# quantumjot/sequitr

Hardware: AMD Instinct MI355X
Metric: segmented Mpixels/sec on 512x512 tiles; IoU vs reference (higher is better)
Workload: dtype f32; 1 GPU; U-Net 2-class inference, launches of 32 512x512x1 tiles, fp32 (BASELINE.json configs[1]: filters 16-32-64-128-256, eltwise_mul bridge); logits + uint8 argmax mask; one 32-tile batch per GPU per step; tiles_this_rank=32

## Files before the change

### sequitr_amd/csrc/sq_common.h

```cpp
#pragma once
#include <hip/hip_runtime.h>
#include <stdint.h>
#include <stdio.h>
#include "../../include/sequitr_hip.h"

typedef float f32x4 __attribute__((ext_vector_type(4)));

#define SQ_NOT_MINE 1

void sq_set_error(const char *fmt, ...);

#define SQ_REQUIRE(cond, ...)            \
    do {                                 \
        if (!(cond)) {                   \
            sq_set_error(__VA_ARGS__);   \
            return SQ_EINVAL;            \
        }                                \
    } while (0)

int sq_plan_bf16_kc(int Cin);
int sq_plan_bf16_bn(int64_t ntiles, int Cout, bool pn, bool mos);
int sq_plan_mosaic_splitk(int Nimg, int h, int w, int Cin, int Cout, int R, int Cc, bool have_ws, int64_t workspace_bytes);
int sq_plan_f32_bn(int64_t ntiles, int Cout);
bool sq_plan_f32_stage32(int bn, int KS, int KC, int Cin, bool concat);
bool sq_plan_l0_takes(int mode, int cout, int act, int H, int W, bool concat, int head_c, bool pooled);
int sq_wgrad_f32_plan(int N, int H, int W, int Cin, int Cout, int K, int64_t *out);

#define SQ_ALIGNED16(p) ((((uintptr_t)(p)) & 15u) == 0)

#define SQ_REQUIRE_ALIGNED(p)                                     \
    do {                                                          \
        if (!SQ_ALIGNED16(p)) {                                   \
            sq_set_error("%s: pointer %s not 16-byte aligned", __func__, #p); \
            return SQ_EALIGN;                                     \
        }                                                         \
    } while (0)

static inline int sq_check_launch(const char *what) {
    hipError_t e = hipGetLastError();
    if (e != hipSuccess) {
        sq_set_error("%s: launch failed: %s", what, hipGetErrorString(e));
        return SQ_ELAUNCH;
    }
    return SQ_OK;
}

__device__ __forceinline__ float sq_act(float v, int act) {
    if (act == SQ_ACT_RELU) return v > 0.0f ? v : 0.0f;
    if (act == SQ_ACT_LEAKY) return v > 0.0f ? v : 0.2f * v;
    return v;
}

__device__ __forceinline__ unsigned sq_xcd_remap(unsigned bid, unsigned nblk) {
    const unsigned q = nblk >> 3, r = nblk & 7u, xcd = bid & 7u, k = bid >> 3;
    const unsigned base = xcd < r ? xcd * (q + 1) : r * (q + 1) + (xcd - r) * q;
    return base + k;
}

struct SqDropKey { unsigned s1, s2; };
__device__ __forceinline__ SqDropKey sq_dropout_key(unsigned seed, const int *__restrict__ step) {
    if (step) seed += (unsigned)step[0] * 0x9E3779B9u;
    SqDropKey k;
    k.s1 = seed * 0x9E3779B1u + 0x7F4A7C15u;
    k.s2 = (seed ^ 0x68E31DA4u) * 0x85EBCA6Bu;
    k.s2 ^= k.s2 >> 13;
    return k;
}
__device__ __forceinline__ unsigned sq_dropout_thr16(float rate) { return (unsigned)(rate * 65536.0f); }
__device__ __forceinline__ unsigned sq_dropout_keep4(SqDropKey k, unsigned q, unsigned thr16) {
    unsigned h = q + k.s1;
    h ^= h >> 16; h *= 0x7FEB352Du; h = h ^ (h >> 15) ^ k.s2; h *= 0x846CA68Bu; h ^= h >> 16;
    unsigned g = (h ^ 0x5BD1E995u) * 0x2C1B3C6Du;
    g ^= g >> 15;
    return (unsigned)((h & 0xFFFFu) >= thr16) | ((unsigned)((h >> 16) >= thr16) << 1) |
           ((unsigned)((g & 0xFFFFu) >= thr16) << 2) | ((unsigned)((g >> 16) >= thr16) << 3);
}

template <int MAXC>
__device__ __forceinline__ float sq_wce_pixel(const float (&zc)[MAXC], const float (&yc)[MAXC], int C, float wp, float g,
                                              float *__restrict__ dz) {
#pragma clang fp contract(off)
    float m = -INFINITY, yt = 0.f, dot = 0.f;
#pragma unroll
    for (int c = 0; c < MAXC; ++c)
        if (c < C) {
            m = zc[c] > m ? zc[c] : m;
            yt += yc[c];
            dot = __builtin_fmaf(yc[c], zc[c], dot);
        }
    float s = 0.f;
#pragma unroll
    for (int c = 0; c < MAXC; ++c)
        if (c < C) s += expf(zc[c] - m);
    const float lse = m + logf(s);
    if (dz) {
#pragma unroll
        for (int c = 0; c < MAXC; ++c)
            if (c < C) dz[c] = g * (expf(zc[c] - lse) * yt - yc[c]);
    }
    return wp * (lse * yt - dot);
}

__device__ __forceinline__ float sq_group_reduce(const float *__restrict__ p, size_t stride, int nblk, int g, int G) {
    float s = 0.f;
    int b = g;
    for (; b + 7 * G < nblk; b += 8 * G) {
        float v[8];
#pragma unroll
        for (int u = 0; u < 8; ++u) v[u] = p[(size_t)(b + u * G) * stride];
#pragma unroll
        for (int u = 0; u < 8; ++u) s += v[u];
    }
    for (; b < nblk; b += G) s += p[(size_t)b * stride];
    for (int m = G >> 1; m > 0; m >>= 1) s += __shfl_xor(s, m);
    return s;
}
static inline int sq_group_size(int nblk) {
    int G = 1;
    while (G < 64 && G * 2 <= nblk) G *= 2;
    return G;
}
```

### sequitr_amd/csrc/sq_conv_epi.h

```cpp
#pragma once
#include "sq_common.h"

struct SqConvEpi {
    float *pooled;
    const float *head_w;
    const float *head_b;
    float *logits;
    uint8_t *mask;
    int head_c;
    int store_y;
    const float *first_w;
    const float *first_b;
    const float *up_x;
    const float *up_w;
    const float *up_b;
    int up_bridge;
    const float *x2;
};

#define SQ_L0_NOT_MINE 1
int sq_conv_l0_launch(int mode, const float *x, const float *w, const float *bias, float *y, int N, int H, int W,
                      int cout, int act, const SqConvEpi &epi, hipStream_t st);
```

### sequitr_amd/csrc/sq_conv_f32_v2.hip

```cpp
#include <stdlib.h>
#include <type_traits>
#include "sq_common.h"
#include "sq_conv_epi.h"

#ifndef SQ_V2_FAST32
#define SQ_V2_FAST32 1
#endif
#ifndef SQ_V2_INNER
#define SQ_V2_INNER 1
#endif
#ifndef SQ_TILE_INTERLEAVE
#define SQ_TILE_INTERLEAVE 1
#endif
#ifndef SQ_STORE_PERMUTE
#define SQ_STORE_PERMUTE 0
#endif


namespace {

constexpr int TH = 16, TW = 16;

template <int BN, int KS, int KC>
struct Cfg2 {
// ... 293 lines not shown
            const float *src = xl + (((hy + 1) >> 1) * C::UP_W + ((hx + 1) >> 1)) * C::UP_PS + kk;
            f32x4 c1 = (f32x4){0.f, 0.f, 0.f, 0.f};
#pragma unroll
            for (int s8 = 0; s8 < 8; ++s8) c1 = __builtin_amdgcn_mfma_f32_16x16x4f32(aw[s8], src[4 * s8], c1, 0, 0, 0);
            const int gy = ty * TH - 1 + hy, gx = tx * TW - 1 + hx;
            const bool inside = (unsigned)gy < (unsigned)H && (unsigned)gx < (unsigned)W;
            if (j < 81) {
                float *d = xs + (hy * C::HALO_W + hx) * C::PS + 4 * kk;
                const float u[4] = {c1[0] + upb.x, c1[1] + upb.y, c1[2] + upb.z, c1[3] + upb.w};
                const float sk[4] = {sr[blk].x, sr[blk].y, sr[blk].z, sr[blk].w};
                float m[4];
#pragma unroll
                for (int e = 0; e < 4; ++e) {
                    const float v = epi.up_bridge == SQ_BRIDGE_ADD ? u[e] + sk[e]
                                  : (epi.up_bridge == SQ_BRIDGE_MUL ? u[e] * sk[e]
                                  : (epi.up_bridge == SQ_BRIDGE_SUB ? u[e] - sk[e] : u[e]));
                    m[e] = inside ? v : 0.f;
                }
                *reinterpret_cast<float2 *>(d) = make_float2(m[0], m[1]);
                *reinterpret_cast<float2 *>(d + 2) = make_float2(m[2], m[3]);
            }
        }
    };

    f32x4 acc[4][NR];
    const float *xb_lds = xs + ((4 * wv) * C::HALO_W + li) * C::PS + kk;
    const float *wa_lds = ws + kk * C::BNS + li;

    auto load_frag = [&](int st, float (&a)[NR], float (&b)[4]) {
        constexpr int SPC = KS * KS * 4;
        const int sub = KC > 16 ? st / SPC : 0, sr = KC > 16 ? st % SPC : st;
        constexpr int Q = KC > 16 ? 4 : KC / 4;
        const int tap = sr / Q, s = sr % Q;
        const int ky = tap / KS, kx = tap % KS;
        const int ch = sub * 16 + s * 4;
#pragma unroll
        for (int nb = 0; nb < NR; ++nb)
            a[nb] = wa_lds[(tap * KC + ch) * C::BNS + ((nb * 16) ^ ((kk & 1) ? C::WSWZ : 0))];
#pragma unroll
        for (int r = 0; r < 4; ++r) b[r] = xb_lds[((r + ky) * C::HALO_W + kx) * C::PS + ch];
    };

    const float slope = act == SQ_ACT_LEAKY ? 0.2f : 1.0f;
    const bool is_relu = act == SQ_ACT_RELU;
    auto actk = [&](float v, auto fastc) {
        if constexpr (decltype(fastc)::value) return __builtin_fmaxf(v, 0.0f);
        else {
            const float neg = is_relu ? 0.0f : v * slope;
            return v > 0.0f ? v : neg;
        }
    };

    float ah[4] = {0.f, 0.f, 0.f, 0.f};
    float hb[4] = {0.f, 0.f, 0.f, 0.f};
    if (epi.head_w) {
#pragma unroll
        for (int s4 = 0; s4 < 4; ++s4) ah[s4] = li < epi.head_c ? epi.head_w[(4 * s4 + kk) * epi.head_c + li] : 0.f;
        if (epi.head_b) {
#pragma unroll
            for (int q = 0; q < 4; ++q) hb[q] = q < epi.head_c ? epi.head_b[q] : 0.f;
        }
    }

#if SQ_STORE_PERMUTE
    const int st_src = (((lane & 3) << 4) | (lane >> 2)) << 2;
    const int st_px = lane >> 2, st_q = lane & 3;
#endif
    float4 bvr[NR];
#pragma unroll
    for (int nb = 0; nb < NR; ++nb) {
        const int co = n0 + nb * 16 + 4 * kk;
        bvr[nb] = (bias && co < Cout) ? *reinterpret_cast<const float4 *>(bias + co) : make_float4(0.f, 0.f, 0.f, 0.f);
    }
    const int fast_lane = (((4 * wv) * W + li) * Cout + 4 * kk) * 4;
    auto epilogue = [&](int tx, int ty, int n, auto fastc) {
        constexpr bool FAST = decltype(fastc)::value;
        auto actf = [&](float v) { return actk(v, fastc); };
        const int gx = tx * TW + li;
#pragma unroll
        for (int nb = 0; nb < NR; ++nb) {
            const int co = n0 + nb * 16 + 4 * kk;
            const float4 bv = bvr[nb];
            f32x4 o[4];
#pragma unroll
            for (int r = 0; r < 4; ++r) {
                const int gy = ty * TH + 4 * wv + r;
                o[r][0] = actf(bias ? acc[r][nb][0] + bv.x : acc[r][nb][0]);
                o[r][1] = actf(bias ? acc[r][nb][1] + bv.y : acc[r][nb][1]);
                o[r][2] = actf(bias ? acc[r][nb][2] + bv.z : acc[r][nb][2]);
                o[r][3] = actf(bias ? acc[r][nb][3] + bv.w : acc[r][nb][3]);
                if (epi.store_y) {
#if SQ_STORE_PERMUTE
                    const float t0 = __int_as_float(__builtin_amdgcn_ds_bpermute(st_src, __float_as_int(o[r][0])));
                    const float t1 = __int_as_float(__builtin_amdgcn_ds_bpermute(st_src, __float_as_int(o[r][1])));
                    const float t2 = __int_as_float(__builtin_amdgcn_ds_bpermute(st_src, __float_as_int(o[r][2])));
                    const float t3 = __int_as_float(__builtin_amdgcn_ds_bpermute(st_src, __float_as_int(o[r][3])));
                    f32x4 t = (f32x4){t0, t1, t2, t3};
                    const int sgx = tx * TW + st_px, sco = n0 + nb * 16 + 4 * st_q;
                    const bool ok = gy < H && sgx < W && sco < Cout;
                    const unsigned off = ok ? (unsigned)((((n * H + gy) * W + sgx) * Cout + sco) * 4) : OOB;
                    __builtin_amdgcn_raw_buffer_store_b128(
                        *reinterpret_cast<__attribute__((__vector_size__(4 * sizeof(unsigned)))) unsigned *>(&t),
                        yrsrc, off, 0, 0);
#else
                    unsigned off;
                    if constexpr (FAST) {
                        off = (unsigned)(fast_lane + nb * 64) + (unsigned)((((n * H + ty * TH + r) * W + tx * TW) * Cout + n0) * 4);
                    } else {
                        const bool ok = gy < H && gx < W && co < Cout;
                        off = ok ? (unsigned)((((n * H + gy) * W + gx) * Cout + co) * 4) : OOB;
                    }
                    __builtin_amdgcn_raw_buffer_store_b128(
                        *reinterpret_cast<__attribute__((__vector_size__(4 * sizeof(unsigned)))) unsigned *>(&o[r]),
                        yrsrc, off, 0, 0);
#endif
                }
                acc[r][nb] = (f32x4){0.f, 0.f, 0.f, 0.f};
            }
            if (epi.pooled) {
#pragma unroll
                for (int pr = 0; pr < 2; ++pr) {
                    float mp[4];
#pragma unroll
                    for (int j = 0; j < 4; ++j) {
                        const float a = o[2 * pr][j], b = o[2 * pr + 1][j];
                        const float v = b > a ? b : a;
                        const float u = __shfl_xor(v, 1);
                        mp[j] = u > v ? u : v;
                    }
                    const int py = (ty * TH + 4 * wv) / 2 + pr, px = gx >> 1;
                    if ((li & 1) == 0 && py < (H >> 1) && px < (W >> 1) && co < Cout)
                        *reinterpret_cast<float4 *>(epi.pooled + ((size_t)(n * (H >> 1) + py) * (W >> 1) + px) * Cout + co) =
                            make_float4(mp[0], mp[1], mp[2], mp[3]);
                }
            }
            if (epi.head_w) {
                float *hs = head_scratch + wv * (16 * C::HEAD_PS);
#pragma unroll
                for (int r = 0; r < 4; ++r) {
                    float *d = hs + li * C::HEAD_PS + 4 * kk;
                    *reinterpret_cast<float2 *>(d) = make_float2(o[r][0], o[r][1]);
                    *reinterpret_cast<float2 *>(d + 2) = make_float2(o[r][2], o[r][3]);
                    __builtin_amdgcn_wave_barrier();
                    f32x4 z = (f32x4){0.f, 0.f, 0.f, 0.f};
#pragma unroll
                    for (int s4 = 0; s4 < 4; ++s4)
                        z = __builtin_amdgcn_mfma_f32_16x16x4f32(ah[s4], hs[li * C::HEAD_PS + 4 * s4 + kk], z, 0, 0, 0);
                    __builtin_amdgcn_wave_barrier();
                    const int gy = ty * TH + 4 * wv + r;
                    if (kk == 0 && gy < H && gx < W) {
                        const size_t p = (size_t)(n * H + gy) * W + gx;
                        float best = 0.f;
                        int bi = 0;
#pragma unroll
                        for (int q = 0; q < 4; ++q)
                            if (q < epi.head_c) {
                                const float v = epi.head_b ? z[q] + hb[q] : z[q];
                                epi.logits[p * epi.head_c + q] = v;
                                if (q == 0 || v > best) { best = v; bi = q; }
                            }
                        if (epi.mask) epi.mask[p] = (uint8_t)bi;
                    }
                }
            }
        }
    };

    const int per_image = tiles_x * tiles_y;
    const int s_n = tstride / per_image, s_y = (tstride % per_image) / tiles_x, s_x = (tstride % per_image) % tiles_x;
    int ctx = t_begin % tiles_x, cty = (t_begin / tiles_x) % tiles_y, cn = t_begin / per_image;
    int ntx = ctx + s_x, nty = cty, nn = cn;
    if (ntx >= tiles_x) { ntx -= tiles_x; nty += 1; }
    nty += s_y;
    if (nty >= tiles_y) { nty -= tiles_y; nn += 1; }
    nn += s_n;
    issue(ctx, cty, cn, 0, true, true);
    __builtin_amdgcn_s_waitcnt(0x0F70);
    commit(true);
#pragma unroll
    for (int r = 0; r < 4; ++r)
#pragma unroll
        for (int nb = 0; nb < NR; ++nb) acc[r][nb] = (f32x4){0.f, 0.f, 0.f, 0.f};
    __syncthreads();
    if constexpr (FIRST) {
        first_conv(ctx, cty);
        __syncthreads();
    }
    if constexpr (UP) {
        up_conv(ctx, cty);
        __syncthreads();
    }

    int tile = t_begin, chunk = 0;
    for (int it = 0; it < nitems; ++it) {
        int ntile = tile, nchk = chunk + 1;
        if (nchk == nchunk) { nchk = 0; ntile = tile + tstride; }
        const bool has_next = it + 1 < nitems;
        const bool same = ntile == tile;
        const int itx = same ? ctx : ntx, ity = same ? cty : nty, itn = same ? cn : nn;
        if (has_next) issue(itx, ity, itn, nchk * KC, restage_w, true);

        {
            float a0[NR], b0[4], a1[NR], b1[4];
            load_frag(0, a0, b0);
            __builtin_amdgcn_s_setprio(0);
#pragma unroll
            for (int st = 0; st < C::NSTEP; st += 2) {
                if (st + 1 < C::NSTEP) load_frag(st + 1, a1, b1);
                __builtin_amdgcn_sched_barrier(0);
#pragma unroll
                for (int r = 0; r < 4; ++r)
#pragma unroll
                    for (int nb = 0; nb < NR; ++nb)
                        acc[r][nb] = __builtin_amdgcn_mfma_f32_16x16x4f32(a0[nb], b0[r], acc[r][nb], 0, 0, 0);
                __builtin_amdgcn_sched_barrier(0);
                if (st + 1 < C::NSTEP) {
                    if (st + 2 < C::NSTEP) load_frag(st + 2, a0, b0);
                    __builtin_amdgcn_sched_barrier(0);
#pragma unroll
                    for (int r = 0; r < 4; ++r)
#pragma unroll
                        for (int nb = 0; nb < NR; ++nb)
                            acc[r][nb] = __builtin_amdgcn_mfma_f32_16x16x4f32(a1[nb], b1[r], acc[r][nb], 0, 0, 0);
                    __builtin_amdgcn_sched_barrier(0);
                }
            }
            __builtin_amdgcn_s_setprio(3);
        }
        __builtin_amdgcn_s_waitcnt(0x0F70);
        if (has_next) {
            __syncthreads();
            commit(restage_w);
            if constexpr (FIRST) {
                __syncthreads();
                first_conv(itx, ity);
            }
            if constexpr (UP) {
                __syncthreads();
                up_conv(itx, ity);
            }
        }
        if (chunk == nchunk - 1) {
            const bool fast = is_relu && cty * TH + TH <= H && ctx * TW + TW <= W && n0 + BN <= Cout;
            if constexpr ((BN == 64 || (SQ_V2_FAST32 && BN == 32 && KC == 32)) && MODE == 0) {
                if (fast) epilogue(ctx, cty, cn, std::integral_constant<bool, true>{});
                else epilogue(ctx, cty, cn, std::integral_constant<bool, false>{});
            } else {
                (void)fast;
                epilogue(ctx, cty, cn, std::integral_constant<bool, false>{});
            }
        }
        if (has_next) __syncthreads();
        if (ntile != tile) {
            ctx = ntx; cty = nty; cn = nn;
            ntx += s_x;
            if (ntx >= tiles_x) { ntx -= tiles_x; nty += 1; }
            nty += s_y;
            if (nty >= tiles_y) { nty -= tiles_y; nn += 1; }
            nn += s_n;
        }
        tile = ntile;
        chunk = nchk;
    }
}

template <int BN, int KS, int KC, int MODE>
int launch_v2(const float *x, const float *w, const float *bias, float *y, int N, int H, int W, int Cin,
              int Cout, float wscale, int act, const SqConvEpi &epi, hipStream_t st) {
    using C = Cfg2<BN, KS, KC>;
    static bool attr_set = false;
    auto kern = conv_mfma_f32_v2_kernel<BN, KS, KC, MODE>;
    constexpr int lds_base = MODE == 1 ? C::LDS_BYTES_FIRST : (MODE == 2 ? C::LDS_BYTES_UP : C::LDS_BYTES);
    constexpr int lds_max = lds_base + C::HEAD_FLOATS * 4;
    const int lds = lds_base + (epi.head_w ? C::HEAD_FLOATS * 4 : 0);
    if (!attr_set) {
        if (hipFuncSetAttribute(reinterpret_cast<const void *>(kern),
                                hipFuncAttributeMaxDynamicSharedMemorySize, lds_max) != hipSuccess) {
            sq_set_error("conv_mfma_f32_v2: cannot reserve %d bytes of LDS", lds_max);
            return SQ_ELAUNCH;
        }
        attr_set = true;
    }
    const int tiles_x = (W + TW - 1) / TW, tiles_y = (H + TH - 1) / TH;
    const int ntiles = tiles_x * tiles_y * N;
    const int gy = (Cout + BN - 1) / BN;
    int want = (256 * (MODE == 2 ? 3 : C::OCC) + gy - 1) / gy;
    if (want < 1) want = 1;
    int tpb = (ntiles + want - 1) / want;
    if (tpb < 1) tpb = 1;
    const int gx = (ntiles + tpb - 1) / tpb;
    hipLaunchKernelGGL(kern, dim3(gx, gy), dim3(256), lds, st, x, w, bias, y, N, H, W, Cin, Cout,
                       wscale, act, tiles_x, tiles_y, ntiles, tpb, epi);
    return sq_check_launch("sq_conv2d_nhwc_fwd_f32(v2)");
}

template <int KS, int KC>
int dispatch_bn(const float *x, const float *w, const float *bias, float *y, int N, int H, int W, int Cin,
                int Cout, float wscale, int act, const SqConvEpi &epi, hipStream_t st) {
    const int ntiles = ((W + TW - 1) / TW) * ((H + TH - 1) / TH) * N;
    const int bn = sq_plan_f32_bn(ntiles, Cout);
    if constexpr (KS == 3 && KC == 16) {
        if (sq_plan_f32_stage32(bn, KS, KC, Cin, epi.x2 != nullptr))
            return launch_v2<32, 3, 32, false>(x, w, bias, y, N, H, W, Cin, Cout, wscale, act, epi, st);
    }
    if (bn == 64) return launch_v2<64, KS, KC, false>(x, w, bias, y, N, H, W, Cin, Cout, wscale, act, epi, st);
    if (bn == 32) return launch_v2<32, KS, KC, false>(x, w, bias, y, N, H, W, Cin, Cout, wscale, act, epi, st);
    return launch_v2<16, KS, KC, false>(x, w, bias, y, N, H, W, Cin, Cout, wscale, act, epi, st);
}

bool fits32(int N, int H, int W, int C) { return (size_t)N * H * W * (size_t)C * 4 < ((size_t)1 << 31); }

}

int sq_conv_mfma_v2(const float *x, const float *w, const float *bias, float *y, int N, int H, int W,
                    int Cin, int Cout, int K, float wscale, int act, hipStream_t st) {
    SqConvEpi epi = {};
    epi.store_y = 1;
    if (Cin == 16 && (Cout == 16 || Cout == 32) && K == 3 && wscale == 1.0f) {
        const int r = sq_conv_l0_launch(0, x, w, bias, y, N, H, W, Cout, act, epi, st);
        if (r != SQ_L0_NOT_MINE) return r;
    }
    if (Cin % 16 == 0)
        return K == 3 ? dispatch_bn<3, 16>(x, w, bias, y, N, H, W, Cin, Cout, wscale, act, epi, st)
                      : dispatch_bn<1, 16>(x, w, bias, y, N, H, W, Cin, Cout, wscale, act, epi, st);
    return K == 3 ? dispatch_bn<3, 8>(x, w, bias, y, N, H, W, Cin, Cout, wscale, act, epi, st)
                  : dispatch_bn<1, 8>(x, w, bias, y, N, H, W, Cin, Cout, wscale, act, epi, st);
}

extern "C" int sq_conv2d_concat_nhwc_fwd_f32(const float *xa, const float *xb, const float *w, const float *bias, float *y,
                                             int N, int H, int W, int Ca, int Cout, int K, int act, void *stream) {
    SQ_REQUIRE(xa && xb && w && y, "sq_conv2d_concat_nhwc_fwd_f32: null tensor pointer");
    SQ_REQUIRE(N > 0 && H > 0 && W > 0 && (K == 1 || K == 3), "sq_conv2d_concat_nhwc_fwd_f32: bad shape / K");
    SQ_REQUIRE(Ca % 16 == 0 && Ca > 0 && Cout % 4 == 0 && Cout > 0,
               "sq_conv2d_concat_nhwc_fwd_f32: channels per source %d (multiple of 16), Cout=%d (multiple of 4)", Ca, Cout);
    SQ_REQUIRE(fits32(N, H, W, 2 * Ca > Cout ? 2 * Ca : Cout), "sq_conv2d_concat_nhwc_fwd_f32: tensors must be < 2 GiB");
    SQ_REQUIRE(act >= SQ_ACT_NONE && act <= SQ_ACT_LEAKY, "sq_conv2d_concat_nhwc_fwd_f32: bad activation %d", act);
    SQ_REQUIRE_ALIGNED(xa); SQ_REQUIRE_ALIGNED(xb); SQ_REQUIRE_ALIGNED(w); SQ_REQUIRE_ALIGNED(y);
    if (bias) SQ_REQUIRE_ALIGNED(bias);
    SqConvEpi epi = {};
    epi.store_y = 1;
    epi.x2 = xb;
    hipStream_t st = reinterpret_cast<hipStream_t>(stream);
    return K == 3 ? dispatch_bn<3, 16>(xa, w, bias, y, N, H, W, 2 * Ca, Cout, 1.0f, act, epi, st)
                  : dispatch_bn<1, 16>(xa, w, bias, y, N, H, W, 2 * Ca, Cout, 1.0f, act, epi, st);
}

extern "C" int sq_conv3x3_pool_fwd_f32(const float *x, const float *w, const float *bias, float *y, float *pooled,
                                       int N, int H, int W, int Cin, int Cout, int act, void *stream) {
    SQ_REQUIRE(x && w && y && pooled, "sq_conv3x3_pool_fwd_f32: null tensor pointer");
    SQ_REQUIRE(N > 0 && H > 0 && W > 0 && H % 2 == 0 && W % 2 == 0, "sq_conv3x3_pool_fwd_f32: H, W must be even");
    SQ_REQUIRE(Cin % 16 == 0 && Cin > 0 && Cout % 4 == 0 && Cout > 0,
               "sq_conv3x3_pool_fwd_f32: Cin=%d (multiple of 16), Cout=%d (multiple of 4)", Cin, Cout);
    SQ_REQUIRE(fits32(N, H, W, Cin > Cout ? Cin : Cout), "sq_conv3x3_pool_fwd_f32: tensors must be < 2 GiB");
    SQ_REQUIRE(act >= SQ_ACT_NONE && act <= SQ_ACT_LEAKY, "sq_conv3x3_pool_fwd_f32: bad activation %d", act);
    SQ_REQUIRE_ALIGNED(x); SQ_REQUIRE_ALIGNED(w); SQ_REQUIRE_ALIGNED(y); SQ_REQUIRE_ALIGNED(pooled);
    if (bias) SQ_REQUIRE_ALIGNED(bias);
    SqConvEpi epi = {};
    epi.store_y = 1;
    epi.pooled = pooled;
    if (Cin == 16 && Cout == 16) {
        const int r = sq_conv_l0_launch(0, x, w, bias, y, N, H, W, 16, act, epi, reinterpret_cast<hipStream_t>(stream));
        if (r != SQ_L0_NOT_MINE) return r;
    }
    return dispatch_bn<3, 16>(x, w, bias, y, N, H, W, Cin, Cout, 1.0f, act, epi, reinterpret_cast<hipStream_t>(stream));
}

extern "C" int sq_conv3x3_head_fwd_f32(const float *x, const float *w, const float *bias, const float *head_w,
                                       const float *head_b, float *logits, uint8_t *mask, int N, int H, int W,
                                       int Cin, int head_c, int act, void *stream) {
    SQ_REQUIRE(x && w && head_w && logits, "sq_conv3x3_head_fwd_f32: null tensor pointer");
    SQ_REQUIRE(N > 0 && H > 0 && W > 0 && Cin % 16 == 0 && Cin > 0, "sq_conv3x3_head_fwd_f32: Cin=%d (multiple of 16)", Cin);
    SQ_REQUIRE(head_c >= 1 && head_c <= 4, "sq_conv3x3_head_fwd_f32: head_c=%d (1..4)", head_c);
    SQ_REQUIRE(fits32(N, H, W, Cin > 16 ? Cin : 16), "sq_conv3x3_head_fwd_f32: tensors must be < 2 GiB");
    SQ_REQUIRE(act >= SQ_ACT_NONE && act <= SQ_ACT_LEAKY, "sq_conv3x3_head_fwd_f32: bad activation %d", act);
    SQ_REQUIRE_ALIGNED(x); SQ_REQUIRE_ALIGNED(w);
    if (bias) SQ_REQUIRE_ALIGNED(bias);
    SqConvEpi epi = {};
    epi.store_y = 0;
    epi.head_w = head_w; epi.head_b = head_b; epi.logits = logits; epi.mask = mask; epi.head_c = head_c;
    if (Cin == 16) {
        const int r = sq_conv_l0_launch(0, x, w, bias, nullptr, N, H, W, 16, act, epi, reinterpret_cast<hipStream_t>(stream));
        if (r != SQ_L0_NOT_MINE) return r;
    }
    return launch_v2<16, 3, 16, false>(x, w, bias, nullptr, N, H, W, Cin, 16, 1.0f, act, epi,
                                       reinterpret_cast<hipStream_t>(stream));
}

extern "C" int sq_conv3x3_first_block_fwd_f32(const float *x, const float *w1, const float *b1, const float *w2,
                                              const float *b2, float *y, float *pooled, int N, int H, int W,
                                              void *stream) {
    SQ_REQUIRE(x && w1 && b1 && w2 && y, "sq_conv3x3_first_block_fwd_f32: null tensor pointer");
    SQ_REQUIRE(N > 0 && H > 0 && W > 0, "sq_conv3x3_first_block_fwd_f32: bad shape");
    SQ_REQUIRE(!pooled || (H % 2 == 0 && W % 2 == 0), "sq_conv3x3_first_block_fwd_f32: pooling needs even H, W");
    SQ_REQUIRE(fits32(N, H, W, 16), "sq_conv3x3_first_block_fwd_f32: tensors must be < 2 GiB");
    SQ_REQUIRE_ALIGNED(w2); SQ_REQUIRE_ALIGNED(y);
    if (b2) SQ_REQUIRE_ALIGNED(b2);
    if (pooled) SQ_REQUIRE_ALIGNED(pooled);
    SqConvEpi epi = {};
    epi.store_y = 1;
    epi.pooled = pooled;
    epi.first_w = w1; epi.first_b = b1;
    {
        const int r = sq_conv_l0_launch(1, x, w2, b2, y, N, H, W, 16, SQ_ACT_RELU, epi, reinterpret_cast<hipStream_t>(stream));
        if (r != SQ_L0_NOT_MINE) return r;
    }
    return launch_v2<16, 3, 16, true>(x, w2, b2, y, N, H, W, 1, 16, 1.0f, SQ_ACT_RELU, epi,
                                      reinterpret_cast<hipStream_t>(stream));
}

extern "C" int sq_convT_conv3x3_fwd_f32(const float *x_low, const float *wt, const float *bt, const float *skip,
                                        int bridge, const float *w, const float *bias, float *y, int N, int H, int W,
                                        int act, void *stream) {
    SQ_REQUIRE(x_low && wt && skip && w && y, "sq_convT_conv3x3_fwd_f32: null tensor pointer");
    SQ_REQUIRE(N > 0 && H > 0 && W > 0 && H % 2 == 0 && W % 2 == 0, "sq_convT_conv3x3_fwd_f32: H, W must be even");
    SQ_REQUIRE(bridge >= SQ_BRIDGE_NONE && bridge <= SQ_BRIDGE_SUB, "sq_convT_conv3x3_fwd_f32: bad bridge %d", bridge);
    SQ_REQUIRE(fits32(N, H, W, 16), "sq_convT_conv3x3_fwd_f32: tensors must be < 2 GiB");
    SQ_REQUIRE(act >= SQ_ACT_NONE && act <= SQ_ACT_LEAKY, "sq_convT_conv3x3_fwd_f32: bad activation %d", act);
    SQ_REQUIRE_ALIGNED(x_low); SQ_REQUIRE_ALIGNED(skip); SQ_REQUIRE_ALIGNED(w); SQ_REQUIRE_ALIGNED(y);
    if (bias) SQ_REQUIRE_ALIGNED(bias);
    if (bt) SQ_REQUIRE_ALIGNED(bt);
    SqConvEpi epi = {};
    epi.store_y = 1;
    epi.up_x = x_low; epi.up_w = wt; epi.up_b = bt; epi.up_bridge = bridge;
    {
        const int r = sq_conv_l0_launch(2, skip, w, bias, y, N, H, W, 16, act, epi, reinterpret_cast<hipStream_t>(stream));
        if (r != SQ_L0_NOT_MINE) return r;
    }
    return launch_v2<16, 3, 16, 2>(skip, w, bias, y, N, H, W, 16, 16, 1.0f, act, epi,
                                   reinterpret_cast<hipStream_t>(stream));
}
```

### sequitr_amd/csrc/sq_conv_plan.hip

```cpp
#include "sq_conv_epi.h"
#include <stdlib.h>

namespace {
constexpr int TILE = 16;
int64_t ntiles_of(int N, int H, int W) { return (int64_t)((W + TILE - 1) / TILE) * ((H + TILE - 1) / TILE) * N; }
}

int sq_plan_bf16_kc(int Cin) { return Cin % 32 == 0 ? 32 : (Cin % 16 == 0 ? 16 : 8); }

int sq_plan_bf16_bn(int64_t ntiles, int Cout, bool pn, bool mos) {
    if (pn) return Cout <= 16 ? 16 : (Cout <= 32 ? 32 : 64);
    int bn = Cout >= 64 ? 64 : (Cout > 16 ? 32 : 16);
    static const int narrow = [] { const char *e = getenv("SQ_CONV_BF16_NARROW"); return e ? atoi(e) : 1; }();
    while (narrow && bn > 16 && ntiles * ((Cout + bn - 1) / bn) < 2 * 256) bn >>= 1;
    static const int force_bn = [] { const char *e = getenv("SQ_MOS_BN"); return e ? atoi(e) : 0; }();
    if (mos && (force_bn == 16 || force_bn == 32 || force_bn == 64) && force_bn <= ((Cout + 15) / 16) * 16) bn = force_bn;
    return bn;
}

int sq_plan_mosaic_splitk(int Nimg, int h, int w, int Cin, int Cout, int R, int Cc, bool have_ws, int64_t workspace_bytes) {
    const int H = R * (h + 1), W = Cc * (w + 1);
    const int nchunk = Cin / sq_plan_bf16_kc(Cin);
    const int64_t blocks = ntiles_of(1, H, W) * ((Cout + 15) / 16);
    const int64_t slice = (int64_t)Nimg * h * w * Cout * 4;
    int S = 1;
    static const int sk_on = [] { const char *e = getenv("SQ_CONV_SPLITK"); return e ? atoi(e) : 1; }();
    if (sk_on && have_ws && Cout % 4 == 0 && blocks < 256 && nchunk >= 4)
        while (S < 8 && nchunk % (2 * S) == 0 && nchunk / (2 * S) >= 2 && blocks * S < 512 && slice * 2 * S <= workspace_bytes) S *= 2;
    static const int force_s = [] { const char *e = getenv("SQ_MOS_S"); return e ? atoi(e) : 0; }();
    if (force_s >= 1 && have_ws && nchunk % force_s == 0 && slice * force_s <= workspace_bytes) S = force_s;
    return S;
}

int sq_plan_f32_bn(int64_t ntiles, int Cout) {
    int bn = Cout >= 64 ? 64 : (Cout > 16 ? 32 : 16);
    while (bn > 16 && ntiles * ((Cout + bn - 1) / bn) < 2 * 256) bn >>= 1;
    return bn;
}

bool sq_plan_f32_stage32(int bn, int KS, int KC, int Cin, bool concat) {
    static const bool on = [] { const char *e = getenv("SQ_CONV_STAGE32"); return !(e && e[0] == '0'); }();
    return KS == 3 && KC == 16 && bn == 32 && Cin % 32 == 0 && !concat && on;
}

bool sq_plan_l0_takes(int mode, int cout, int act, int H, int W, bool concat, int head_c, bool pooled) {
    if (cout != 16 && !(cout == 32 && mode == 0 && !head_c && !pooled)) return false;
    const char *e = getenv("SQ_CONV_L0");
    if (e && e[0] == '0') return false;
    if (act != SQ_ACT_RELU || H % 16 != 0 || W % 16 != 0 || concat) return false;
    if (head_c && head_c != 2) return false;
    if (head_c && pooled) return false;
    return true;
}

extern "C" int sq_conv_plan(int family, int form, int N, int H, int W, int Cin, int Cout, int K, int act, int flags,
                            const int *mosaic, int64_t workspace_bytes, int *out) {
    SQ_REQUIRE(out, "sq_conv_plan: null out");
    SQ_REQUIRE(N > 0 && H > 0 && W > 0 && Cin > 0 && Cout > 0 && (K == 1 || K == 3), "sq_conv_plan: bad shape / K");
    SQ_REQUIRE(act >= SQ_ACT_NONE && act <= SQ_ACT_LEAKY, "sq_conv_plan: bad activation %d", act);
    out[0] = out[1] = out[2] = 0;
    out[3] = 1;
    out[4] = 0;
    if (family == SQ_PLAN_F32) {
        SQ_REQUIRE(!mosaic, "sq_conv_plan: the f32 family has no mosaic form");
        SQ_REQUIRE(Cout % 4 == 0 && (Cin % 16 == 0 || (Cin == 8 && form == SQ_PLAN_PLAIN)),
                   "sq_conv_plan: the f32 v2 kernels take Cin %% 16 == 0 (or 8, plain), Cout %% 4 == 0");
        SQ_REQUIRE(form == SQ_PLAN_PLAIN || form == SQ_PLAN_CONCAT || (form == SQ_PLAN_POOL && K == 3),
                   "sq_conv_plan: f32 form %d at K=%d does not exist", form, K);
        const bool wscale1 = !(flags & SQ_PLAN_WSCALE);
        const bool offer = form == SQ_PLAN_PLAIN ? (Cin == 16 && (Cout == 16 || Cout == 32) && K == 3 && wscale1)
                                                 : (form == SQ_PLAN_POOL && Cin == 16 && Cout == 16);
        if (offer && sq_plan_l0_takes(0, Cout, act, H, W, false, 0, form == SQ_PLAN_POOL)) {
            out[0] = Cout;
            out[1] = 16;
            out[2] = 1;
            out[4] = 1;
            return SQ_OK;
        }
        const int KC = Cin % 16 == 0 ? 16 : 8;
        const int bn = sq_plan_f32_bn(ntiles_of(N, H, W), Cout);
        const bool s32 = sq_plan_f32_stage32(bn, K, KC, Cin, form == SQ_PLAN_CONCAT);
        out[0] = bn;
        out[1] = s32 ? 32 : KC;
        out[2] = (Cout + bn - 1) / bn;
        return SQ_OK;
    }
    SQ_REQUIRE(family == SQ_PLAN_BF16 || family == SQ_PLAN_MIXED, "sq_conv_plan: bad family %d", family);
    SQ_REQUIRE(Cin % 8 == 0 && Cout % 4 == 0, "sq_conv_plan: Cin=%d (multiple of 8), Cout=%d (multiple of 4)", Cin, Cout);
    const bool bf = family == SQ_PLAN_BF16;
    int NN = N, HH = H, WW = W;
    if (mosaic) {
        SQ_REQUIRE(K == 3 && (form == SQ_PLAN_PLAIN || form == SQ_PLAN_ACTGATE), "sq_conv_plan: the mosaic forms are 3x3 plain / act-gated");
        SQ_REQUIRE(mosaic[0] > 0 && mosaic[1] > 0 && (int64_t)mosaic[0] * mosaic[1] >= N && H <= 8 && W <= 8,
                   "sq_conv_plan: mosaic of R x Cc >= Nimg cells of images up to 8 x 8");
        NN = 1;
        HH = mosaic[0] * (H + 1);
        WW = mosaic[1] * (W + 1);
        if (bf) out[3] = sq_plan_mosaic_splitk(N, H, W, Cin, Cout, mosaic[0], mosaic[1], workspace_bytes > 0, workspace_bytes);
    } else {
        switch (form) {
        case SQ_PLAN_PLAIN: case SQ_PLAN_ACTGATE: break;
        case SQ_PLAN_POOL: case SQ_PLAN_JUNCTION:
            SQ_REQUIRE(bf && K == 3, "sq_conv_plan: form %d is a 3x3 form on bf16 tensors", form); break;
        case SQ_PLAN_MASK: case SQ_PLAN_MASKGATE:
            SQ_REQUIRE(bf && K == 3 && Cout % 16 == 0, "sq_conv_plan: the mask forms are 3x3, Cout %% 16 == 0, bf16 tensors"); break;
        case SQ_PLAN_PIXELNORM:
            SQ_REQUIRE(bf && K == 3 && Cout % 8 == 0 && Cout <= 64, "sq_conv_plan: the pixel-norm form is 3x3, Cout %% 8 == 0, <= 64"); break;
        case SQ_PLAN_FIRSTBLOCK:
            SQ_REQUIRE(bf && K == 3 && Cin == 16 && Cout == 16, "sq_conv_plan: the first block is the 3x3 16 -> 16 conv"); break;
        default:
            SQ_REQUIRE(false, "sq_conv_plan: form %d does not exist in family %d", form, family);
        }
    }
    const int bn = sq_plan_bf16_bn(ntiles_of(NN, HH, WW), Cout, form == SQ_PLAN_PIXELNORM, mosaic != nullptr);
    out[0] = bn;
    out[1] = sq_plan_bf16_kc(Cin);
    out[2] = (Cout + bn - 1) / bn;
    return SQ_OK;
}
```

Before: 1646 Mpixels/s.

## Add specialized 64-wide f32 3x3 conv kernel with double-buffered halo staging

Result: no change. 1652 Mpixels/s, median of 6 (+0.4%).

```diff
diff --git a/sequitr_amd/csrc/sq_common.h b/sequitr_amd/csrc/sq_common.h
--- a/sequitr_amd/csrc/sq_common.h
+++ b/sequitr_amd/csrc/sq_common.h
@@ -24,6 +24,7 @@
 int sq_plan_f32_bn(int64_t ntiles, int Cout);
 bool sq_plan_f32_stage32(int bn, int KS, int KC, int Cin, bool concat);
 bool sq_plan_l0_takes(int mode, int cout, int act, int H, int W, bool concat, int head_c, bool pooled);
+bool sq_plan_w64_takes(int bn, int kc, int K, int N, int H, int W, int Cin, int Cout, int act, bool wscale1, bool concat);
 int sq_wgrad_f32_plan(int N, int H, int W, int Cin, int Cout, int K, int64_t *out);
 
 #define SQ_ALIGNED16(p) ((((uintptr_t)(p)) & 15u) == 0)
diff --git a/sequitr_amd/csrc/sq_conv_epi.h b/sequitr_amd/csrc/sq_conv_epi.h
--- a/sequitr_amd/csrc/sq_conv_epi.h
+++ b/sequitr_amd/csrc/sq_conv_epi.h
@@ -21,3 +21,5 @@
 #define SQ_L0_NOT_MINE 1
 int sq_conv_l0_launch(int mode, const float *x, const float *w, const float *bias, float *y, int N, int H, int W,
                       int cout, int act, const SqConvEpi &epi, hipStream_t st);
+int sq_conv_w64_launch(const float *x, const float *w, const float *bias, float *y, float *pooled, int N, int H, int W,
+                       int Cin, int Cout, hipStream_t st);
diff --git a/sequitr_amd/csrc/sq_conv_f32_v2.hip b/sequitr_amd/csrc/sq_conv_f32_v2.hip
--- a/sequitr_amd/csrc/sq_conv_f32_v2.hip
+++ b/sequitr_amd/csrc/sq_conv_f32_v2.hip
@@ -619,6 +619,8 @@
     if constexpr (KS == 3 && KC == 16) {
         if (sq_plan_f32_stage32(bn, KS, KC, Cin, epi.x2 != nullptr))
             return launch_v2<32, 3, 32, false>(x, w, bias, y, N, H, W, Cin, Cout, wscale, act, epi, st);
+        if (epi.store_y && !epi.head_w && sq_plan_w64_takes(bn, KC, KS, N, H, W, Cin, Cout, act, wscale == 1.0f, epi.x2 != nullptr))
+            return sq_conv_w64_launch(x, w, bias, y, epi.pooled, N, H, W, Cin, Cout, st);
     }
     if (bn == 64) return launch_v2<64, KS, KC, false>(x, w, bias, y, N, H, W, Cin, Cout, wscale, act, epi, st);
     if (bn == 32) return launch_v2<32, KS, KC, false>(x, w, bias, y, N, H, W, Cin, Cout, wscale, act, epi, st);
diff --git a/sequitr_amd/csrc/sq_conv_f32_w64.hip b/sequitr_amd/csrc/sq_conv_f32_w64.hip
--- /dev/null
+++ b/sequitr_amd/csrc/sq_conv_f32_w64.hip
@@ -0,0 +1,264 @@
+#include <stdlib.h>
+#include "sq_common.h"
+#include "sq_conv_epi.h"
+
+#ifndef SQ_W64_SETPRIO
+#define SQ_W64_SETPRIO 1
+#endif
+
+#ifndef SQ_W64_DBUF
+#define SQ_W64_DBUF 1
+#endif
+
+namespace {
+
+constexpr int TH = 16, TW = 16, HWD = 18, HP = HWD * HWD;
+constexpr int PS = 24;
+constexpr int XS_FLOATS = HP * PS;
+constexpr int XITEMS = HP * 4, XSLOTS = 6;
+constexpr int BN = 64, KC = 16;
+constexpr unsigned OOB = 0x80000000u;
+
+enum { EPI_STORE = 0, EPI_POOL = 1 };
+
+struct W64Args {
+    const float *x, *w, *bias;
+    float *y, *pooled;
+    int N, H, W, Cin, Cout;
+    int tiles_x, tiles_y, ntiles;
+};
+
+typedef unsigned u32x4 __attribute__((__vector_size__(4 * sizeof(unsigned))));
+
+__device__ __forceinline__ float relu(float v) { return __builtin_fmaxf(v, 0.0f); }
+
+template <int EPI>
+__global__ __launch_bounds__(256, 2) void conv_w64_kernel(const W64Args a) {
+    extern __shared__ __attribute__((aligned(16))) float smem[];
+    float *xs = smem;
+
+    const int tid = threadIdx.x, lane = tid & 63, wv = tid >> 6;
+    const int li = lane & 15, kk = lane >> 4;
+    const int H = a.H, W = a.W, Cin = a.Cin, Cout = a.Cout;
+    const int n0 = blockIdx.y * BN;
+    const int G = (int)gridDim.x;
+    const int vb = (int)sq_xcd_remap(blockIdx.x, gridDim.x);
+    if (vb >= a.ntiles) return;
+    const int t_count = (a.ntiles - vb + G - 1) / G;
+    const int nchunk = Cin / KC;
+    const int nitems = t_count * nchunk;
+    const bool restage_w = nchunk > 1;
+
+    const __amdgpu_buffer_rsrc_t xrsrc = __builtin_amdgcn_make_buffer_rsrc(
+        const_cast<float *>(a.x), 0, (int)((size_t)a.N * H * W * Cin * 4), 0x00020000);
+    const __amdgpu_buffer_rsrc_t wrsrc = __builtin_amdgcn_make_buffer_rsrc(
+        const_cast<float *>(a.w), 0, 9 * Cin * Cout * 4, 0x00020000);
+    const __amdgpu_buffer_rsrc_t yrsrc = __builtin_amdgcn_make_buffer_rsrc(
+        a.y, 0, (int)((size_t)a.N * H * W * Cout * 4), 0x00020000);
+
+    float4 xr[XSLOTS];
+    int xrel[XSLOTS], xpp[XSLOTS];
+#pragma unroll
+    for (int sl = 0; sl < XSLOTS; ++sl) {
+        const int idx = tid + sl * 256, pix = idx >> 2, q = idx & 3;
+        const int py = pix / HWD, px = pix % HWD;
+        xrel[sl] = idx < XITEMS ? ((py * W + px) * Cin + q * 4) * 4 : (int)OOB;
+        xpp[sl] = (py << 8) | px;
+    }
+    auto issue_halo = [&](int tx, int ty, int n, int cc) {
+        const int x0 = tx * TW - 1, y0 = ty * TH - 1;
+        const int base = (((n * H + y0) * W + x0) * Cin + cc) * 4;
+        const bool inner = tx > 0 && tx < a.tiles_x - 1 && ty > 0 && ty < a.tiles_y - 1;
+        if (inner) {
+#pragma unroll
+            for (int sl = 0; sl < XSLOTS; ++sl) {
+                const auto v = __builtin_amdgcn_raw_buffer_load_b128(xrsrc, xrel[sl], base, 0);
+                xr[sl] = *reinterpret_cast<const float4 *>(&v);
+            }
+        } else {
+#pragma unroll
+            for (int sl = 0; sl < XSLOTS; ++sl) {
+                const int py = xpp[sl] >> 8, px = xpp[sl] & 255;
+                const bool inb = (unsigned)(y0 + py) < (unsigned)H && (unsigned)(x0 + px) < (unsigned)W && xrel[sl] != (int)OOB;
+                const unsigned off = inb ? (unsigned)(base + xrel[sl]) : OOB;
+                const auto v = __builtin_amdgcn_raw_buffer_load_b128(xrsrc, off, 0, 0);
+                xr[sl] = *reinterpret_cast<const float4 *>(&v);
+            }
+        }
+    };
+    float *cw = xs + (tid >> 2) * PS + (tid & 3);
+    auto commit_halo = [&](int xoff) {
+#pragma unroll
+        for (int sl = 0; sl < XSLOTS; ++sl) {
+            if (sl < XSLOTS - 1 || tid < XITEMS - (XSLOTS - 1) * 256) {
+                float *d = cw + xoff + sl * 64 * PS;
+                d[0] = xr[sl].x; d[4] = xr[sl].y; d[8] = xr[sl].z; d[12] = xr[sl].w;
+            }
+        }
+    };
+
+    float af[9][4], wr[9][4];
+    int wvo[4];
+#pragma unroll
+    for (int s = 0; s < 4; ++s) wvo[s] = ((4 * s + kk) * Cout + n0 + 16 * wv + li) * 4;
+    auto issue_w = [&](int cc) {
+#pragma unroll
+        for (int t = 0; t < 9; ++t) {
+            const int soff = ((t * Cin + cc) * Cout) * 4;
+#pragma unroll
+            for (int s = 0; s < 4; ++s)
+                wr[t][s] = __builtin_bit_cast(float, __builtin_amdgcn_raw_buffer_load_b32(wrsrc, wvo[s], soff, 0));
+        }
+    };
+    auto take_w = [&]() {
+#pragma unroll
+        for (int t = 0; t < 9; ++t)
+#pragma unroll
+            for (int s = 0; s < 4; ++s) af[t][s] = wr[t][s];
+    };
+    const float4 bv = a.bias ? *reinterpret_cast<const float4 *>(a.bias + n0 + 16 * wv + 4 * kk) : make_float4(0.f, 0.f, 0.f, 0.f);
+
+    f32x4 acc[TH];
+    const float *xb0 = xs + li * PS + 4 * kk;
+    auto mfma_phase = [&](int xoff) {
+        const float *xb = xb0 + xoff;
+        float4 bq[2][3];
+#pragma unroll
+        for (int kx = 0; kx < 3; ++kx) bq[0][kx] = *reinterpret_cast<const float4 *>(xb + kx * PS);
+#if SQ_W64_SETPRIO
+        __builtin_amdgcn_s_setprio(0);
+#endif
+#pragma unroll
+        for (int h = 0; h < HWD; ++h) {
+            if (h + 1 < HWD) {
+#pragma unroll
+                for (int kx = 0; kx < 3; ++kx)
+                    bq[(h + 1) & 1][kx] = *reinterpret_cast<const float4 *>(xb + ((h + 1) * HWD + kx) * PS);
+            }
+            __builtin_amdgcn_sched_barrier(0);
+#pragma unroll
+            for (int kx = 0; kx < 3; ++kx) {
+                const float4 q = bq[h & 1][kx];
+                const float b[4] = {q.x, q.y, q.z, q.w};
+#pragma unroll
+                for (int s = 0; s < 4; ++s) {
+#pragma unroll
+                    for (int ky = 2; ky >= 0; --ky) {
+                        const int r = h - ky;
+                        if (r < 0 || r >= TH) continue;
+                        acc[r] = __builtin_amdgcn_mfma_f32_16x16x4f32(af[ky * 3 + kx][s], b[s], acc[r], 0, 0, 0);
+                    }
+                }
+            }
+            __builtin_amdgcn_sched_barrier(0);
+        }
+#if SQ_W64_SETPRIO
+        __builtin_amdgcn_s_setprio(3);
+#endif
+    };
+
+    const int Hl = H >> 1, Wl = W >> 1;
+    const __amdgpu_buffer_rsrc_t prsrc = __builtin_amdgcn_make_buffer_rsrc(
+        a.pooled, 0, EPI == EPI_POOL ? (int)((size_t)a.N * Hl * Wl * Cout * 4) : 0, 0x00020000);
+    const int yvoff = (li * Cout + n0 + 16 * wv + 4 * kk) * 4;
+    const int pvoff = ((li >> 1) * Cout + n0 + 16 * wv + 4 * kk) * 4;
+    auto epilogue = [&](int tx, int ty, int n) {
+        int yoff = yvoff + (((n * H + ty * TH) * W + tx * TW) * Cout) * 4;
+        int poff = pvoff + (((n * Hl + ty * (TH / 2)) * Wl + tx * (TW / 2)) * Cout) * 4;
+#pragma unroll
+        for (int p = 0; p < TH / 2; ++p) {
+            f32x4 o[2];
+#pragma unroll
+            for (int e = 0; e < 2; ++e) {
+                const int r = 2 * p + e;
+                o[e] = (f32x4){relu(acc[r][0] + bv.x), relu(acc[r][1] + bv.y), relu(acc[r][2] + bv.z), relu(acc[r][3] + bv.w)};
+                __builtin_amdgcn_raw_buffer_store_b128(*reinterpret_cast<const u32x4 *>(&o[e]), yrsrc, yoff, 0, 0);
+                yoff += W * Cout * 4;
+                acc[r] = (f32x4){0.f, 0.f, 0.f, 0.f};
+            }
+            if constexpr (EPI == EPI_POOL) {
+                f32x4 mp;
+#pragma unroll
+                for (int j = 0; j < 4; ++j) {
+                    const float v = __builtin_fmaxf(o[0][j], o[1][j]);
+                    const float u = __builtin_bit_cast(float, __builtin_amdgcn_mov_dpp(__builtin_bit_cast(int, v), 0xB1, 0xF, 0xF, true));
+                    mp[j] = __builtin_fmaxf(u, v);
+                }
+                __builtin_amdgcn_raw_buffer_store_b128(*reinterpret_cast<const u32x4 *>(&mp), prsrc,
+                                                       (li & 1) ? (int)OOB : poff, 0, 0);
+                poff += Wl * Cout * 4;
+            }
+        }
+    };
+
+    const int per_image = a.tiles_x * a.tiles_y;
+    const int s_n = G / per_image, s_y = (G % per_image) / a.tiles_x, s_x = (G % per_image) % a.tiles_x;
+    int ctx = vb % a.tiles_x, cty = (vb / a.tiles_x) % a.tiles_y, cn = vb / per_image;
+    int chunk = 0;
+    issue_halo(ctx, cty, cn, 0);
+    issue_w(0);
+    __builtin_amdgcn_s_waitcnt(0x0F70);
+    commit_halo(0);
+    take_w();
+    int xoff = 0;
+#pragma unroll
+    for (int r = 0; r < TH; ++r) acc[r] = (f32x4){0.f, 0.f, 0.f, 0.f};
+    __syncthreads();
+    for (int it = 0; it < nitems; ++it) {
+        const bool has_next = it + 1 < nitems;
+        const bool last_chunk = chunk == nchunk - 1;
+        int itx = ctx, ity = cty, itn = cn, nchk = chunk + 1;
+        if (last_chunk) {
+            nchk = 0;
+            itx += s_x;
+            if (itx >= a.tiles_x) { itx -= a.tiles_x; ity += 1; }
+            ity += s_y;
+            if (ity >= a.tiles_y) { ity -= a.tiles_y; itn += 1; }
+            itn += s_n;
+        }
+        if (has_next) {
+            issue_halo(itx, ity, itn, nchk * KC);
+            if (restage_w) issue_w(nchk * KC);
+        }
+        mfma_phase(xoff);
+        __builtin_amdgcn_s_waitcnt(0x0F70);
+#if SQ_W64_DBUF
+        xoff = XS_FLOATS - xoff;
+#endif
+        if (has_next) {
+#if !SQ_W64_DBUF
+            __syncthreads();
+#endif
+            commit_halo(xoff);
+            if (restage_w) take_w();
+        }
+        if (last_chunk) epilogue(ctx, cty, cn);
+        if (has_next) __syncthreads();
+        ctx = itx; cty = ity; cn = itn;
+        chunk = nchk;
+    }
+}
+
+template <int EPI>
+int launch_w64(W64Args a, hipStream_t st) {
+    a.tiles_x = a.W / TW;
+    a.tiles_y = a.H / TH;
+    a.ntiles = a.tiles_x * a.tiles_y * a.N;
+    const int gy = a.Cout / BN;
+    int want = (256 * 2 + gy - 1) / gy;
+    int tpb = (a.ntiles + want - 1) / want;
+    if (tpb < 1) tpb = 1;
+    const int gx = (a.ntiles + tpb - 1) / tpb;
+    hipLaunchKernelGGL(conv_w64_kernel<EPI>, dim3(gx, gy), dim3(256), XS_FLOATS * 4 * (SQ_W64_DBUF ? 2 : 1), st, a);
+    return sq_check_launch("conv_w64");
+}
+
+}
+
+int sq_conv_w64_launch(const float *x, const float *w, const float *bias, float *y, float *pooled, int N, int H, int W,
+                       int Cin, int Cout, hipStream_t st) {
+    W64Args a = {};
+    a.x = x; a.w = w; a.bias = bias; a.y = y; a.pooled = pooled;
+    a.N = N; a.H = H; a.W = W; a.Cin = Cin; a.Cout = Cout;
+    return pooled ? launch_w64<EPI_POOL>(a, st) : launch_w64<EPI_STORE>(a, st);
+}
diff --git a/sequitr_amd/csrc/sq_conv_plan.hip b/sequitr_amd/csrc/sq_conv_plan.hip
--- a/sequitr_amd/csrc/sq_conv_plan.hip
+++ b/sequitr_amd/csrc/sq_conv_plan.hip
@@ -1,5 +1,9 @@
 #include "sq_conv_epi.h"
 #include <stdlib.h>
+
+#ifndef SQ_W64_DEFAULT
+#define SQ_W64_DEFAULT 1
+#endif
 
 namespace {
 constexpr int TILE = 16;
@@ -51,6 +55,15 @@
     if (head_c && head_c != 2) return false;
     if (head_c && pooled) return false;
     return true;
+}
+
+bool sq_plan_w64_takes(int bn, int kc, int K, int N, int H, int W, int Cin, int Cout, int act, bool wscale1, bool concat) {
+    if (bn != 64 || kc != 16 || K != 3) return false;
+    const char *e = getenv("SQ_CONV_W64");
+    if (e ? e[0] == '0' : !SQ_W64_DEFAULT) return false;
+    if (Cin % 16 != 0 || Cout % 64 != 0 || H % 16 != 0 || W % 16 != 0) return false;
+    if (act != SQ_ACT_RELU || !wscale1 || concat) return false;
+    return (int64_t)N * H * W * (Cin > Cout ? Cin : Cout) * 4 < ((int64_t)1 << 31);
 }
 
 extern "C" int sq_conv_plan(int family, int form, int N, int H, int W, int Cin, int Cout, int K, int act, int flags,
```
